# tlepoint/fhe.rs

Hardware: NVIDIA H100
Metric: bfv_ct_mul_relin_per_sec_n32768_14x62bit (higher is better)
Workload: dtype u64

## Files before the change

fhe_rs_b200/_capi.py:

```python
from __future__ import annotations

import ctypes as C
import os

_HERE = os.path.dirname(os.path.abspath(__file__))
LIB_PATH = os.environ.get("FHE_B200_LIB") or os.path.join(_HERE, "libfhe_b200.so")

OK = 0
INVALID_ARGUMENT, INVALID_MODULUS, INVALID_DEGREE, NTT_UNAVAILABLE = -1, -2, -3, -4
CONTEXT_MISMATCH, INVALID_LEVEL, BAD_POLY_COUNT, INVALID_REPRESENTATION = -5, -6, -7, -8
NO_MORE_CONTEXT, INVALID_EXPONENT, UNSUPPORTED = -9, -10, -11
CUDA_ERROR, OUT_OF_MEMORY, NO_DEVICE = -20, -21, -22
POWER_BASIS, NTT = 0, 1
ENCODING_POLY, ENCODING_SIMD = 0, 1

_u32, _u64, _vp, _i = C.c_uint32, C.c_uint64, C.c_void_p, C.c_int
_pu32, _pu64, _pu8 = C.POINTER(C.c_uint32), C.POINTER(C.c_uint64), C.POINTER(C.c_uint8)
_pp = C.POINTER(C.c_void_p)
SYMBOLS = {
    "fhe_b200_version": (C.c_char_p, []),
    "fhe_b200_last_error": (C.c_char_p, []),
    "fhe_b200_params_create": (_i, [_i, _u32, _vp, _u32, _vp, _u32, _vp, _pp]),
    "fhe_b200_params_create_from_sizes": (_i, [_i, _u32, _vp, _u32, _vp, _u32, _pp]),
    "fhe_b200_params_destroy": (_i, [_vp]),
# ... 67 lines not shown
    "fhe_b200_expand": (_i, [_vp, _u32, _pp, _u32, _vp, _vp]),
    "fhe_b200_substitute": (_i, [_vp, _u32, _vp, _vp]),
    "fhe_b200_switch_down": (_i, [_vp, _vp]),
    "fhe_b200_key_switch": (_i, [_vp, _u32, _vp, _vp, _vp]),
    "fhe_b200_key_switch_keyed": (_i, [_vp, _u32, _pp, _u32, _pu32, _vp, _vp]),
    "fhe_b200_relinearize_keyed": (_i, [_vp, _pp, _u32, _pu32, _vp, _vp]),
    "fhe_b200_mul_relin_keyed": (_i, [_vp, _vp, _pp, _u32, _pu32, _i, _vp, _vp]),
    "fhe_b200_galois_keyed": (_i, [_vp, _u32, _pp, _u32, _pu32, _vp, _vp]),
    "fhe_b200_expand_keyed": (_i, [_vp, _u32, _pp, _u32, _u32, _pu32, _vp, _vp]),
    "fhe_b200_galois_many": (_i, [_vp, _pu32, _pp, _pu32, _u32, _pu32, _vp, _vp]),
    "fhe_b200_inner_sum": (_i, [_vp, _pp, _u32, _vp, _vp]),
    "fhe_b200_inner_sum_keyed": (_i, [_vp, _pp, _u32, _u32, _pu32, _vp, _vp]),
    "fhe_b200_scale": (_i, [_vp, _i, _vp, _vp]),
    "fhe_b200_poly_packed_bytes": (_i, [_vp, _u32, C.POINTER(C.c_size_t)]),
    "fhe_b200_batch_packed_bytes": (_i, [_vp, C.POINTER(C.c_size_t)]),
    "fhe_b200_batch_pack": (_i, [_vp, _u32, _u32, _vp, _vp]),
    "fhe_b200_batch_unpack": (_i, [_vp, _u32, _u32, _vp, _vp]),
    "fhe_b200_transcode": (_i, [_vp, _vp, _u32, C.c_size_t, C.c_size_t, _u32, _vp, _u32, C.c_size_t, C.c_size_t,
                                _u32, _u32, _vp]),
    "fhe_b200_fold": (_i, [_vp, _u32, _u32, _vp, _vp]),
    "fhe_b200_sync": (_i, [_vp]),
    "fhe_b200_launch_count": (_u64, []),
    "fhe_b200_debug_scaler_tables": (_i, [_vp, _u32, _i, _pu32, _pu32, _pu32] + [_vp] * 8),
    "fhe_b200_debug_ntt_tables": (_i, [_vp, _u64, _vp, _vp, _vp, _vp, _pu64]),
    "fhe_b200_debug_expansion_monomial": (_i, [_vp, _u32, _u32, _vp]),
    "fhe_b200_debug_encoder_tables": (_i, [_vp, _u32, _vp, _vp, _vp, _pu64, _vp]),
}

_lib = None


def lib() -> C.CDLL:
    global _lib
    if _lib is None:
        if not os.path.exists(LIB_PATH):
            raise ImportError(
                "fhe_rs_b200: %s is missing -- build it with `python -m fhe_rs_b200.build` "
                "(there is no CPU fallback)" % LIB_PATH)
        _lib = C.CDLL(LIB_PATH)
        for name, (res, args) in SYMBOLS.items():
            f = getattr(_lib, name)
            f.restype, f.argtypes = res, args
    return _lib


class FheError(RuntimeError):
# ... 9 lines not shown
```

fhe_rs_b200/csrc/capi.cu:

```cuda
#include <algorithm>
#include <atomic>
#include <cstring>
#include <functional>
#include <map>
#include <memory>
#include <mutex>
#include <string>
#include <vector>

#include "../../include/fhe_b200.h"
#include "engine.hpp"
#include "host/precompute.hpp"

using namespace fhe_b200;

namespace {

thread_local std::string g_last_error;

struct ScalerData {
  ScalerTablesH h;
  ScalerDev dev;
};

// ... 76 lines not shown
  d.tg_lo = s.h.theta_gamma_lo; d.tg_hi = s.h.theta_gamma_hi; d.tg_sign = s.h.theta_gamma_sign;
  for (size_t j = 0; j < to_moduli.size(); j++) d.to_ids[j] = (unsigned short)prime_index(limb_primes, to_moduli[j]);
  d.all_solinas = switches().no_solinas ? 0 : 1;
  for (u64 q : to_moduli)
    if ((q >> 61) != 1 || ((1ull << 62) - q) >= (1ull << 28)) d.all_solinas = 0;
  d.gamma = tables.put(s.h.gamma);
  d.omega = tables.put(s.h.omega);
  d.to_lo = tables.put(s.h.theta_omega_lo);
  d.to_hi = tables.put(s.h.theta_omega_hi);
  d.to_sign = tables.put(s.h.theta_omega_sign);
  std::vector<unsigned char> order;
  d.n_pos = 0;
  for (int sg = 0; sg < 2; sg++)
    for (size_t i = 0; i < s.h.theta_omega_sign.size(); i++)
      if ((int)s.h.theta_omega_sign[i] == sg && (s.h.theta_omega_lo[i] | s.h.theta_omega_hi[i]) != 0) {
        order.push_back((unsigned char)i);
        d.n_pos += sg == 0;
      }
  d.n_terms = (u32)order.size();
  if (order.empty()) order.push_back(0);
  d.to_order = tables.put(order);
  d.tgar_lo = tables.put(s.h.theta_garner_lo);
  d.tgar_hi = tables.put(s.h.theta_garner_hi);
}

LimbDev make_limb_dev(u64 q, const NttTablesH& t, DeviceTables& tables) {
  ModulusH m(q);
  LimbDev d;
  std::memset(&d, 0, sizeof(d));
  d.p = q; d.p2 = 2 * q; d.bhi = m.bhi; d.blo = m.blo; d.c128 = m.c128;
  d.ninv = t.ninv; d.zn = t.zn;
  const u64 cc = (1ull << 62) - q;
  const bool sol = (q >> 61) == 1 && cc < (1ull << 28) && !switches().no_solinas;
  const bool sol_ntt = switches().solinas_ntt;
  auto pairs = [&](const std::vector<u64>& v, const std::vector<u64>& shoup) {
    std::vector<ulonglong2> o(v.size());
    for (size_t k = 0; k < v.size(); k++) {
      o[k].x = v[k];
      o[k].y = (sol && sol_ntt) ? (u64)((((u128)v[k]) << 32) % q) : shoup[k];
    }
    return o;
  };
  d.sol_c = sol ? cc : 0;
  d.sol_ntt = (sol && sol_ntt) ? 1 : 0;
  d.ninv_s = (sol && sol_ntt) ? (u64)((((u128)t.ninv) << 32) % q) : t.ninv_s;
  d.zn_s = (sol && sol_ntt) ? (u64)((((u128)t.zn) << 32) % q) : t.zn_s;
// ... 463 lines not shown
}

void galois_range(const fhe_b200_params* par, const LevelData& lv, const KeySet& gk, const u64* src, u32 src0, u64* dst,
                  u32 n, bool sum, cudaStream_t st) {
  const size_t row = (size_t)1 << par->logn, L = lv.L;
  std::vector<u32> exps(n), source(n);
  for (u32 c = 0; c < n; c++) {
    exps[c] = gk.exps[gk.key_of(c)];
    source[c] = gk.source ? gk.source[c] : src0 + c;
  }
  Workspace ws(par, st);
  u64* s = sum ? nullptr : ws.words((size_t)n * 2 * L * row);
  u64* c2 = ws.words((size_t)n * L * row);
  launch_substitute_ntt(src, 2 * L * row, sum ? dst : s, 2 * L * row, c2, L * row, exps.data(), source.data(), n,
                        (u32)L, sum, lv.ctx_ids, par->d_limbs, par->logn, st);
  launch_ntt(c2, c2, n * (u32)L, lv.ctx_ids, par->d_limbs, par->logn, true, 1, false, st);
  key_switch_apply(par, gk, c2, n, dst, sum ? 1 : 2, s, ws, st);
}

void mul_core(const fhe_b200_params* par, const LevelData& lv, const u64* a, const u64* b, u32 cts, u64* out0,
              u64* out1, int split, Workspace& ws, cudaStream_t st) {
  const u32 L = lv.L, E = lv.E, K = lv.K, logn = par->logn;
  const size_t row = (size_t)1 << logn;
  u64* A_l = ws.words((size_t)cts * 2 * L * row);
  u64* A_r = ws.words((size_t)cts * 2 * L * row);
  u64* X_l = ws.words((size_t)cts * 2 * E * row);
  u64* X_r = ws.words((size_t)cts * 2 * E * row);
  u64* T = ws.words((size_t)cts * 3 * K * row);
  launch_ntt(a, A_l, cts * 2 * L, lv.ctx_ids, par->d_limbs, logn, true, 1, false, st);
  launch_ntt(b, A_r, cts * 2 * L, lv.ctx_ids, par->d_limbs, logn, true, 1, false, st);
  launch_scale(lv.ext.dev, par->d_limbs, A_l, X_l, nullptr, cts * 2, E, L, E, 0, logn, st);
  launch_scale(lv.ext.dev, par->d_limbs, A_r, X_r, nullptr, cts * 2, E, L, E, 0, logn, st);
  launch_ntt(X_l, X_l, cts * 2 * E, lv.ext_ids, par->d_limbs, logn, false, 1, false, st);
  launch_ntt(X_r, X_r, cts * 2 * E, lv.ext_ids, par->d_limbs, logn, false, 1, false, st);
  if (!launch_tensor_inverse_ntt(a, b, X_l, X_r, T, cts, L, K, lv.mul_ids, par->d_limbs, logn, st)) {
    launch_tensor(a, b, X_l, X_r, T, cts, L, L, L, K, lv.mul_ids, par->d_limbs, logn, st);
    launch_ntt(T, T, cts * 3 * K, lv.mul_ids, par->d_limbs, logn, true, 1, false, st);
  }
  launch_scale(lv.down.dev, par->d_limbs, T, out0, out1, cts * 3, L, 0, L, split, logn, st);
}

void mul_core_parts(const fhe_b200_params* par, const LevelData& lv, const u64* a, u32 na, const u64* b, u32 nb, u32 cts,
                    u64* out, Workspace& ws, cudaStream_t st) {
  const u32 L = lv.L, E = lv.E, K = lv.K, logn = par->logn, nc = na + nb - 1;
  const size_t row = (size_t)1 << logn;
  const u64* src[2] = {a, b};
  const u32 np[2] = {na, nb};
  u64* X[2];
  for (int s = 0; s < 2; s++) {
    u64* pb = ws.words((size_t)cts * np[s] * L * row);
    X[s] = ws.words((size_t)cts * np[s] * E * row);
    launch_ntt(src[s], pb, cts * np[s] * L, lv.ctx_ids, par->d_limbs, logn, true, 1, false, st);
    launch_scale(lv.ext.dev, par->d_limbs, pb, X[s], nullptr, cts * np[s], E, L, E, 0, logn, st);
    launch_ntt(X[s], X[s], cts * np[s] * E, lv.ext_ids, par->d_limbs, logn, false, 1, false, st);
  }
  u64* T = ws.words((size_t)cts * nc * K * row);
  launch_tensor_nm(a, b, X[0], X[1], T, cts, L, E, na, nb, lv.mul_ids, par->d_limbs, logn, st);
// ... 2224 lines not shown
  const LevelData& lv = par->level(out->level);
  const u32 L = lv.L, logn = par->logn, count = ct->count;
  ChunkRunner chunks(par, count, (cudaStream_t)stream, std::max<u32>(1, chunk_size() / (u32)P));
  chunks.run([&](u32 c0, u32 n, cudaStream_t st) {
    Workspace ws(par, st);
    u64* coeffs = ws.words((P * n) << logn);
    launch_fold_stage(ct->d + c0 * ct->words_per_ct(), n, ct->parts, row_words, in_bits, out_bits, (u32)P, coeffs, logn,
                      st);
    for (size_t i = 0; i < P; i++)
      launch_ntt(coeffs + ((i * n) << logn), out->d + ((i * count + c0) * L << logn), n * L, lv.ctx_ids, par->d_limbs,
                 logn, false, L, true, st);
  });
  FHE_CUDA(cudaGetLastError());
  out->repr = FHE_B200_NTT;
  API_END
}

int fhe_b200_sync(void* stream) {
  API_BEGIN
  FHE_CUDA(cudaStreamSynchronize((cudaStream_t)stream));
  API_END
}

int fhe_b200_debug_scaler_tables(const fhe_b200_params* p, uint32_t level, int which, uint32_t* n_from, uint32_t* n_to,
                                 uint32_t* shift, uint64_t* gamma, uint64_t* omega, uint64_t* theta_gamma,
                                 uint64_t* theta_omega_lo, uint64_t* theta_omega_hi, uint8_t* theta_omega_sign,
                                 uint64_t* theta_garner_lo, uint64_t* theta_garner_hi) {
  API_BEGIN
  REQUIRE(p, FHE_B200_INVALID_ARGUMENT, "null argument");
  const LevelData& lv = p->level(level);
  REQUIRE(which >= 0 && which <= 2, FHE_B200_INVALID_ARGUMENT, "which must be 0, 1 or 2");
  const ScalerTablesH& h = which == 0 ? lv.ext.h : which == 1 ? lv.down.h : lv.plain.h;
  if (n_from) *n_from = h.n_from;
  if (n_to) *n_to = h.n_to;
  if (shift) *shift = h.shift;
  auto cp = [](uint64_t* dst, const std::vector<u64>& v) {
    if (dst) for (size_t i = 0; i < v.size(); i++) dst[i] = v[i];
  };
  cp(gamma, h.gamma);
  cp(omega, h.omega);
  if (theta_gamma) { theta_gamma[0] = h.theta_gamma_lo; theta_gamma[1] = h.theta_gamma_hi; theta_gamma[2] = h.theta_gamma_sign; }
  cp(theta_omega_lo, h.theta_omega_lo);
  cp(theta_omega_hi, h.theta_omega_hi);
  if (theta_omega_sign) for (size_t i = 0; i < h.theta_omega_sign.size(); i++) theta_omega_sign[i] = h.theta_omega_sign[i];
  cp(theta_garner_lo, h.theta_garner_lo);
  cp(theta_garner_hi, h.theta_garner_hi);
// ... 52 lines not shown
```

fhe_rs_b200/csrc/engine.hpp:

```cpp
#pragma once
#include <atomic>
#include <cuda.h>
#include <cuda_runtime.h>
#include <vector>

#include "ntt.cuh"

namespace fhe_b200 {

extern std::atomic<unsigned long long> g_launches;

struct Switches {
  enum Ntt { NTT_FAST, NTT_AUTO, NTT_TMA };
  enum Ksmac { KSMAC_FUSED, KSMAC_TMA, KSMAC_CLASSIC };
  u32 chunk;
  u32 streams;
  Ntt ntt;
  bool generic_ntt;
  bool solinas_ntt;
  bool no_solinas;
  bool no_tensor_fusion;
  bool classic_scaler;
  Ksmac ksmac;
  int tma_cols;
// ... 48 lines not shown
void launch_dot(const u64* ct, const u64* pt, u64* out, u32 groups, u32 n_terms, u32 parts, u32 ct_count,
                u32 pt_count, const RowIds& ids, const LimbDev* limbs, u32 logn, cudaStream_t st);

void launch_tensor(const u64* a, const u64* b, const u64* xa, const u64* xb, u64* out, u32 cts, u32 L, u32 nca,
                   u32 ncb, u32 K, const RowIds& mul_ids, const LimbDev* limbs, u32 logn, cudaStream_t st);

void launch_tensor_nm(const u64* a, const u64* b, const u64* xa, const u64* xb, u64* out, u32 cts, u32 L, u32 E, u32 na,
                      u32 nb, const RowIds& mul_ids, const LimbDev* limbs, u32 logn, cudaStream_t st);

struct ScalerDev {
  u32 n_from, n_to, is_one, shift;
  u64 tg_lo, tg_hi;
  u32 tg_sign;
  u32 all_solinas;
  const u64* gamma;
  const u64* omega;
  const u64* to_lo;
  const u64* to_hi;
  const unsigned char* to_sign;
  const unsigned char* to_order;
  u32 n_pos, n_terms;
  const u64* tgar_lo;
  const u64* tgar_hi;
  unsigned short to_ids[kMaxPos];
};
void launch_scale(const ScalerDev& S, const LimbDev* limbs, const u64* in, u64* out0, u64* out1, u32 polys,
                  u32 out_rows_per_poly, u32 start, u32 n_out, int split3, u32 logn, cudaStream_t st);

constexpr u32 kKeyPairs = 64;
constexpr u32 kKeySlots = 512;
struct KeyTable {
  const u64* k0[kKeyPairs];
  const u64* k1[kKeyPairs];
  u32 n;
  unsigned char slot[kKeySlots];
};
struct KeyRange {
  u32 ct0, cts;
  KeyTable keys;
};
#ifdef __CUDACC__
__device__ __forceinline__ u32 key_slot(const KeyTable& K, u32 ct) { return K.n > 1 ? K.slot[ct] : 0; }
#endif

void launch_ksmac(const u64* inter, const std::vector<KeyRange>& ranges, const u64* base0, const u64* base1, u64* out0,
                  u64* out1, u32 n_dig, u32 Lk, u32 out_ct_rows, const RowIds& ids, const LimbDev* limbs, u32 logn,
                  cudaStream_t st, bool adjacent = false);

// ... 96 lines not shown
```

fhe_rs_b200/csrc/host/precompute.hpp:

```cpp
#pragma once
#include <cstdint>
#include <stdexcept>
#include <string>
#include <vector>

#include "bigint.hpp"

namespace fhe_b200 {

typedef unsigned long long u64;
typedef unsigned __int128 u128;

struct FheError : std::runtime_error {
  int code;
  FheError(int c, const std::string& m) : std::runtime_error(m), code(c) {}
};

inline u64 mulmod_h(u64 a, u64 b, u64 p) { return (u64)((u128)a * b % p); }
inline u64 powmod_h(u64 a, u64 e, u64 p) {
  u64 r = 1 % p;
  a %= p;
  while (e) {
    if (e & 1) r = mulmod_h(r, a, p);
    a = mulmod_h(a, a, p);
// ... 107 lines not shown
  BigUint product;
  std::vector<BigUint> garner;
  explicit RnsContextH(const std::vector<u64>& q) : moduli(q), product(1) {
    if (q.empty()) throw FheError(-2, "EmptyModuli");
    for (u64 m : q) product = product * BigUint(m);
    for (u64 m : q) {
      BigUint q_star = product / BigUint(m);
      u64 q_tilde;
      if (!invmod_h(q_star.mod_u64(m), m, &q_tilde)) throw FheError(-2, "NonCoprimeModuli");
      garner.push_back(q_star * BigUint(q_tilde));
    }
  }
};

struct ScalerTablesH {
  uint32_t n_from = 0, n_to = 0, is_one = 0, shift = 0;
  std::vector<u64> gamma;
  u64 theta_gamma_lo = 0, theta_gamma_hi = 0;
  uint32_t theta_gamma_sign = 0;
  std::vector<u64> omega;
  std::vector<u64> theta_omega_lo, theta_omega_hi;
  std::vector<uint8_t> theta_omega_sign;
  std::vector<u64> theta_garner_lo, theta_garner_hi;
};

inline void extract_projection_and_theta(const std::vector<u64>& to, const BigUint& input, const BigUint& num,
                                         const BigUint& den, bool round_up, std::vector<u64>* projected,
                                         u64* lo, u64* hi, bool* sign) {
  BigUint ni = num * input;
  BigUint gamma = (ni + (den >> 1)) / den;
  projected->clear();
  for (u64 m : to) projected->push_back(gamma.mod_u64(m));
  BigUint theta = ni % den;
  bool s = false;
  if (den > BigUint(1)) {
    if (den.is_odd()) {
      if (theta > (den >> 1)) { s = true; theta = den - theta; }
    } else if (theta >= (den >> 1)) { s = true; theta = den - theta; }
  }
  if (round_up) {
    theta = s ? (theta << 127) / den : ((theta << 127) + den - BigUint(1)) / den;
  } else {
    theta = s ? ((theta << 127) + den - BigUint(1)) / den : (theta << 127) / den;
  }
  u128 v = theta.low_u128();
  *lo = (u64)v;
// ... 1 lines not shown
  *sign = s;
}

inline ScalerTablesH make_scaler_tables(const RnsContextH& from, const RnsContextH& to, const BigUint& num,
                                        const BigUint& den) {
  if (den.is_zero()) throw FheError(-1, "scaling factor denominator is zero");
  ScalerTablesH t;
  t.n_from = (uint32_t)from.moduli.size();
  t.n_to = (uint32_t)to.moduli.size();
  t.is_one = num == den;
  bool sg;
  extract_projection_and_theta(to.moduli, from.product, num, den, false, &t.gamma, &t.theta_gamma_lo,
                               &t.theta_gamma_hi, &sg);
  t.theta_gamma_sign = sg;
  t.omega.assign((size_t)t.n_to * t.n_from, 0);
  t.theta_omega_lo.resize(t.n_from);
  t.theta_omega_hi.resize(t.n_from);
  t.theta_omega_sign.resize(t.n_from);
  for (uint32_t i = 0; i < t.n_from; i++) {
    std::vector<u64> proj;
    extract_projection_and_theta(to.moduli, from.garner[i], num, den, true, &proj, &t.theta_omega_lo[i],
                                 &t.theta_omega_hi[i], &sg);
    t.theta_omega_sign[i] = sg;
    for (uint32_t j = 0; j < t.n_to; j++) t.omega[(size_t)j * t.n_from + i] = proj[j] % to.moduli[j];
  }
  uint32_t shift = 127;
  for (u64 qi : from.moduli) {
    u128 v = (u128)qi * t.n_from;
    uint32_t lg = 0;
    while (((u128)1 << lg) < v) lg++;
    uint32_t s = 192 - 1 - lg;
    if (s < shift) shift = s;
  }
  t.shift = shift;
  t.theta_garner_lo.resize(t.n_from);
  t.theta_garner_hi.resize(t.n_from);
  for (uint32_t i = 0; i < t.n_from; i++) {
    BigUint theta = ((from.garner[i] << shift) + (from.product >> 1)) / from.product;
    u128 v = theta.low_u128();
    t.theta_garner_lo[i] = (u64)v;
    t.theta_garner_hi[i] = (u64)(v >> 64);
  }
  return t;
}

}
```

fhe_rs_b200/csrc/kernels.cu:

```cuda
#include <algorithm>
#include <cstdint>
#include <cstdlib>
#include <cstring>
#include <vector>

#include "engine.hpp"
#include "ntt_tma.cuh"

namespace fhe_b200 {

typedef unsigned __int128 u128;

namespace {

struct EwArgs {
  u64* a;
  const u64* b;
  size_t n_words;
  u32 logn, limbs_per_poly;
  const LimbDev* limbs;
  unsigned short ids[kMaxPos];
};

template <int OP>
// ... 387 lines not shown
      u64 y = acc[k].reduce(M);
      u64* dst;
      if (A.split3) {
        u32 ct = poly / 3, part = poly % 3;
        dst = part < 2 ? A.out0 + ((((size_t)ct * 2 + part) * n_out + jj) << A.logn)
                       : A.out1 + (((size_t)ct * n_out + jj) << A.logn);
      } else {
        dst = A.out0 + (((size_t)poly * A.out_rows_per_poly + jj) << A.logn);
      }
      dst[c0 + cc] = y;
    }
  }
}


struct ScaleTmaArgs {
  ScalerDev S;
  const LimbDev* limbs;
  u64 *out0, *out1;
  u32 polys, out_rows_per_poly, start, n_out, split3, logn;
  u32 tiles_total;
};

template <bool IS_ONE, int UNR>
__global__ void __launch_bounds__(kScaleTC) scale_tma_kernel(const __grid_constant__ CUtensorMap tm_in, const ScaleTmaArgs A) {
  using namespace tma;
  extern __shared__ __align__(128) u64 smem[];
  const ScalerDev& S = A.S;
  const u32 nf = S.n_from, n_out = A.n_out;
  const u32 n_out4 = (n_out + 3) & ~3u;
  constexpr u32 TC = kScaleTC;
  u64* s_r = smem;
  u32* s_omega = reinterpret_cast<u32*>(s_r + (size_t)nf * TC);
  u64* s_gamma = reinterpret_cast<u64*>(s_omega + (size_t)nf * 3 * n_out4);
  u64* s_p2 = s_gamma + n_out4;
  u64* s_c = s_p2 + n_out4;
  u64* s_tgl = s_c + n_out4;
  u64* s_tgh = s_tgl + nf;
  u64* s_tol = s_tgh + nf;
  u64* s_toh = s_tol + nf;
  u32* s_ord = reinterpret_cast<u32*>(s_toh + nf);
  u64* s_bar = reinterpret_cast<u64*>(s_ord + ((nf + 1) & ~1u));
  const u32 bar = smem_u32(s_bar);
  const u32 cc = threadIdx.x;

  stage_omega_split(s_omega, S, A.start, n_out, n_out4);
  for (u32 i = cc; i < n_out4; i += TC) {
    const bool live = i < n_out;
    const LimbDev& M = A.limbs[S.to_ids[A.start + (live ? i : 0)]];
    s_gamma[i] = live ? S.gamma[A.start + i] : 0;
    s_p2[i] = M.p2;
    s_c[i] = M.sol_c;
  }
  for (u32 i = cc; i < nf; i += TC) {
    s_tgl[i] = S.tgar_lo[i];
    s_tgh[i] = S.tgar_hi[i];
    const u32 src = (!IS_ONE && i < S.n_terms) ? S.to_order[i] : 0;
    s_tol[i] = IS_ONE ? 0 : S.to_lo[src];
    s_toh[i] = IS_ONE ? 0 : S.to_hi[src];
    s_ord[i] = src * TC * 8;
  }
  if (cc == 0) {
    mbar_init(bar, 1);
    asm volatile("fence.mbarrier_init.release.cluster;" ::: "memory");
  }
  __syncthreads();

  const u32 N = 1u << A.logn;
  const u32 per_poly = N / TC;
  const u32 dst_r = smem_u32(s_r);
  const u32 tile_bytes = nf * TC * 8;
  u32 tile = blockIdx.x;
  if (cc == 0 && tile < A.tiles_total) {
    mbar_expect_tx(bar, tile_bytes);
    load_2d(dst_r, &tm_in, (tile % per_poly) * TC, (tile / per_poly) * nf, bar);
  }
  const u32 my_r = dst_r + cc * 8;
  for (u32 it = 0; tile < A.tiles_total; tile += gridDim.x, it++) {
    const u32 poly = tile / per_poly;
    const u32 c0 = (tile - poly * per_poly) * TC;
    mbar_wait(bar, it & 1);

    u128 v;
    {
      AccTheta at;
      at.clear();
#pragma unroll 2
      for (u32 i = 0; i < nf; i++) at.mac(lds64(my_r + i * TC * 8), s_tgl[i], s_tgh[i]);
      u32 acc[7];
      at.words(acc);
      U256 sg = u256_from_acc(acc);
      const u32 bs = S.shift - 1 - 64;
      u64 lo = (sg.w1 >> bs) | (sg.w2 << (64 - bs));
      u64 hi = (sg.w2 >> bs) | (sg.w3 << (64 - bs));
      u128 x = ((u128)hi << 64) | lo;
      v = (x >> 1) + (x & 1);
    }
    bool w_sign = false;
    u128 w = 0;
    if (!IS_ONE) {
      U256 s_pos = {0, 0, 0, 0}, s_neg = {0, 0, 0, 0};
#pragma unroll 1
      for (u32 sg = 0; sg < 2; sg++) {
        AccTheta at;
        at.clear();
        const u32 k0 = sg ? S.n_pos : 0, k1 = sg ? S.n_terms : S.n_pos;
#pragma unroll 2
        for (u32 k = k0; k < k1; k++) at.mac(lds64(my_r + s_ord[k]), s_tol[k], s_toh[k]);
        u32 wds[7];
        at.words(wds);
        if (sg == 0) s_pos = u256_from_acc(wds);
        else s_neg = u256_from_acc(wds);
      }
      U256 so = u256_sub(s_pos, s_neg);
      U256 vt = u256_mul_128(v, S.tg_lo, S.tg_hi);
      so = S.tg_sign ? u256_add(so, vt) : u256_sub(so, vt);
      w_sign = (so.w3 != 0) || (so.w2 >> 63);
      if (w_sign) {
        u64 n1 = ~so.w1, n2 = ~so.w2, n3 = ~so.w3;
        u128 y = ((u128)((n2 >> 62) | (n3 << 2)) << 64) | ((n1 >> 62) | (n2 << 2));
        w = (y + 1) >> 1;
      } else {
        u128 y = ((u128)((so.w2 >> 62) | (so.w3 << 2)) << 64) | ((so.w1 >> 62) | (so.w2 << 2));
        w = (y >> 1) + (y & 1);
      }
    }
    const u64 mask62 = (1ull << 62) - 1;
    const u64 vl = (u64)v & mask62, wl = (u64)w & mask62;
    const u32 vh = (u32)(v >> 62), wh = (u32)(w >> 62);

    u64* dst;
    size_t dstride = (size_t)1 << A.logn;
    if (A.split3) {
      const u32 ct = poly / 3, part = poly - ct * 3;
      dst = part < 2 ? A.out0 + ((((size_t)ct * 2 + part) * n_out) << A.logn) : A.out1 + (((size_t)ct * n_out) << A.logn);
    } else {
      dst = A.out0 + (((size_t)poly * A.out_rows_per_poly) << A.logn);
    }
    dst += c0 + cc;

    for (u32 j0 = 0; j0 < n_out; j0 += 4) {
      AccKara acc[4];
#pragma unroll
      for (int k = 0; k < 4; k++) acc[k].clear();
      const u32* om = s_omega + j0;
      const u32 g = min(4u, n_out - j0);
      switch (g) {
        case 4: scale_mac_group<4, UNR>(acc, s_r + cc, om, nf, n_out4); break;
        case 3: scale_mac_group<3, UNR>(acc, s_r + cc, om, nf, n_out4); break;
        case 2: scale_mac_group<2, UNR>(acc, s_r + cc, om, nf, n_out4); break;
// ... 7 lines not shown
          load_2d(dst_r, &tm_in, (nxt % per_poly) * TC, (nxt / per_poly) * nf, bar);
        }
      }
#pragma unroll
      for (int k = 0; k < 4; k++) {
        const u32 jj = j0 + k;
        if (jj >= n_out) break;
        const u64 p2 = s_p2[jj];
        const u32 c = (u32)s_c[jj];
        acc[k].mac(split31(csub(p2 - ((u64)vh * c + vl), p2 >> 1)), split31(s_gamma[jj]));
        if (!IS_ONE) {
          const u64 wr = (u64)wh * c + wl;
          acc[k].add64(w_sign ? p2 - wr : wr);
        }
        u64 lo, mid;
        u32 hi32;
        acc[k].merged(lo, mid, hi32);
        dst[(size_t)jj * dstride] = csub(fold192_solinas(lo, mid, hi32, c), p2 >> 1);
      }
    }
  }
}

__global__ void scale_small_kernel(ScaleArgs A) {
  const ScalerDev& S = A.S;
  const u32 nf = S.n_from, n_out = A.n_out;
  const u32 N = 1u << A.logn;
  const u32 idx = blockIdx.x * blockDim.x + threadIdx.x;
  if (idx >= A.polys * N) return;
  const u32 poly = idx >> A.logn, c = idx & (N - 1);
  const u64* src = A.in + (((size_t)poly * nf) << A.logn) + c;
  u32 av[7] = {0, 0, 0, 0, 0, 0, 0}, ap[7] = {0, 0, 0, 0, 0, 0, 0}, an[7] = {0, 0, 0, 0, 0, 0, 0};
  for (u32 i = 0; i < nf; i++) {
    const u64 r = src[(size_t)i << A.logn];
    mac_theta(av, r, S.tgar_lo[i], S.tgar_hi[i]);
    if (!S.is_one) {
      if (S.to_sign[i]) mac_theta(an, r, S.to_lo[i], S.to_hi[i]);
      else mac_theta(ap, r, S.to_lo[i], S.to_hi[i]);
    }
  }
  U256 sg = u256_from_acc(av);
  const u32 bs = S.shift - 1 - 64;
  u64 lo = (sg.w1 >> bs) | (sg.w2 << (64 - bs));
  u64 hi = (sg.w2 >> bs) | (sg.w3 << (64 - bs));
  u128 x = ((u128)hi << 64) | lo;
  u128 v = (x >> 1) + (x & 1);
// ... 1080 lines not shown
  A.cts = cts; A.L = L; A.E = E; A.na = na; A.nb = nb; A.logn = logn;
  A.limbs = limbs;
  copy_ids(A.ids, mul_ids);
  size_t total = ((size_t)cts * (na + nb - 1) * (L + E)) << logn;
  if (!total) return;
  tensor_nm_kernel<<<(unsigned)((total + 255) / 256), 256, 0, st>>>(A);
  g_launches++;
}

static bool launch_scale_tma(const ScalerDev& S, const LimbDev* limbs, const u64* in, u64* out0, u64* out1, u32 polys,
                             u32 out_rows_per_poly, u32 start, u32 n_out, int split3, u32 logn, cudaStream_t st) {
  if (switches().classic_scaler || !tensor_map_encoder() || logn < 7 || (reinterpret_cast<uintptr_t>(in) & 127))
    return false;
  const u32 N = 1u << logn, nf = S.n_from;
  if (nf > 64 || (u64)polys * nf >= (1ull << 31)) return false;
  CUtensorMap tm;
  if (!box_map(&tm, in, (u64)polys * nf, logn, kScaleTC, nf)) return false;
  ScaleTmaArgs A;
  A.S = S; A.limbs = limbs; A.out0 = out0; A.out1 = out1;
  A.polys = polys; A.out_rows_per_poly = out_rows_per_poly; A.start = start; A.n_out = n_out;
  A.split3 = split3; A.logn = logn;
  A.tiles_total = polys * (N / kScaleTC);
  const size_t n_out4 = (n_out + 3) & ~(size_t)3;
  const size_t smem = (nf * kScaleTC + 3 * n_out4 + 4 * nf) * sizeof(u64) + nf * 3 * n_out4 * sizeof(u32) +
                      ((nf + 1) & ~(size_t)1) * 4 + 16;
  auto resident = [&](const void* k) {
    ensure_dynamic_smem(k, smem);
    int per_sm = 0;
    FHE_CUDA(cudaOccupancyMaxActiveBlocksPerMultiprocessor(&per_sm, k, kScaleTC, smem));
    return (u32)std::min<u64>(A.tiles_total, (u64)sm_count() * std::max(per_sm, 1));
  };
  if (switches().scale_unroll == 4) {
    if (S.is_one) scale_tma_kernel<true, 4><<<resident((const void*)scale_tma_kernel<true, 4>), kScaleTC, smem, st>>>(tm, A);
    else scale_tma_kernel<false, 4><<<resident((const void*)scale_tma_kernel<false, 4>), kScaleTC, smem, st>>>(tm, A);
  } else {
    if (S.is_one) scale_tma_kernel<true, 2><<<resident((const void*)scale_tma_kernel<true, 2>), kScaleTC, smem, st>>>(tm, A);
    else scale_tma_kernel<false, 2><<<resident((const void*)scale_tma_kernel<false, 2>), kScaleTC, smem, st>>>(tm, A);
  }
  g_launches++;
  return true;
}

void launch_scale(const ScalerDev& S, const LimbDev* limbs, const u64* in, u64* out0, u64* out1, u32 polys,
                  u32 out_rows_per_poly, u32 start, u32 n_out, int split3, u32 logn, cudaStream_t st) {
  if (!polys || !n_out) return;
  if (S.all_solinas &&
      launch_scale_tma(S, limbs, in, out0, out1, polys, out_rows_per_poly, start, n_out, split3, logn, st))
    return;
  ScaleArgs A;
  A.S = S; A.limbs = limbs; A.in = in; A.out0 = out0; A.out1 = out1;
  A.polys = polys; A.out_rows_per_poly = out_rows_per_poly; A.start = start; A.n_out = n_out;
  A.split3 = split3; A.logn = logn;
  const u32 N = 1u << logn;
  if (N < (u32)kScaleTC) {
    const u32 total = polys * N;
    scale_small_kernel<<<(total + 63) / 64, 64, 0, st>>>(A);
    g_launches++;
    return;
  }
  const size_t n_out4 = (n_out + 3) & ~(size_t)3, nf = S.n_from;
  const size_t smem = (nf * kScaleTC + n_out4 + 5 * nf) * sizeof(u64) + nf * 3 * n_out4 * sizeof(u32);
  ensure_dynamic_smem((const void*)scale_kernel, smem);
  scale_kernel<<<polys * (N / kScaleTC), kScaleTC, smem, st>>>(A);
// ... 168 lines not shown
```

include/fhe_b200.h:

```cpp
#ifndef FHE_B200_H
#define FHE_B200_H

#include <stddef.h>
#include <stdint.h>

#ifdef __cplusplus
extern "C" {
#endif

typedef enum {
  FHE_B200_OK = 0,
  FHE_B200_INVALID_ARGUMENT = -1,
  FHE_B200_INVALID_MODULUS = -2,
  FHE_B200_INVALID_DEGREE = -3,
  FHE_B200_NTT_UNAVAILABLE = -4,
  FHE_B200_CONTEXT_MISMATCH = -5,
  FHE_B200_INVALID_LEVEL = -6,
  FHE_B200_BAD_POLY_COUNT = -7,
  FHE_B200_INVALID_REPRESENTATION = -8,
  FHE_B200_NO_MORE_CONTEXT = -9,
  FHE_B200_INVALID_EXPONENT = -10,
  FHE_B200_UNSUPPORTED = -11,
  FHE_B200_CUDA_ERROR = -20,
  FHE_B200_OUT_OF_MEMORY = -21,
// ... 156 lines not shown
                             const uint32_t* set_index, fhe_b200_batch* out, void* stream);
int fhe_b200_scale(const fhe_b200_batch* in, int which, fhe_b200_batch* out, void* stream);
int fhe_b200_batch_alloc_mul_basis(const fhe_b200_params* p, uint32_t count, uint32_t parts, uint32_t level,
                                   int repr, fhe_b200_batch** out);

int fhe_b200_poly_packed_bytes(const fhe_b200_params* p, uint32_t level, size_t* nbytes);
int fhe_b200_batch_packed_bytes(const fhe_b200_batch* b, size_t* nbytes);
int fhe_b200_batch_pack(const fhe_b200_batch* b, uint32_t first, uint32_t n, uint8_t* host_out, void* stream);
int fhe_b200_batch_unpack(fhe_b200_batch* b, uint32_t first, uint32_t n, const uint8_t* host_in, void* stream);

int fhe_b200_transcode(const fhe_b200_params* p, const void* in, uint32_t in_elem, size_t in_len, size_t in_stride,
                       uint32_t in_bits, void* out, uint32_t out_elem, size_t out_len, size_t out_stride,
                       uint32_t out_bits, uint32_t n_rows, void* stream);
int fhe_b200_fold(const fhe_b200_batch* ct, uint32_t in_bits, uint32_t out_bits, fhe_b200_batch* out, void* stream);

int fhe_b200_sync(void* stream);
uint64_t fhe_b200_launch_count(void);

int fhe_b200_debug_scaler_tables(const fhe_b200_params* p, uint32_t level, int which, uint32_t* n_from,
                                 uint32_t* n_to, uint32_t* shift, uint64_t* gamma, uint64_t* omega,
                                 uint64_t* theta_gamma , uint64_t* theta_omega_lo,
                                 uint64_t* theta_omega_hi, uint8_t* theta_omega_sign,
                                 uint64_t* theta_garner_lo, uint64_t* theta_garner_hi);
int fhe_b200_debug_ntt_tables(const fhe_b200_params* p, uint64_t q, uint64_t* omegas, uint64_t* omegas_shoup,
                              uint64_t* zetas_inv, uint64_t* zetas_inv_shoup, uint64_t* size_inv);
int fhe_b200_debug_expansion_monomial(const fhe_b200_params* p, uint32_t level, uint32_t l, uint64_t* out);
int fhe_b200_debug_encoder_tables(const fhe_b200_encoder* e, uint32_t level, uint32_t* index_map, uint64_t* omegas,
                                  uint64_t* zetas_inv, uint64_t* q_mod_t, uint64_t* delta);

#ifdef __cplusplus
}
#endif
#endif
```

Baseline: 3831.

## Use Karatsuba-split accumulation with float fractional estimate in TMA scaler, exact fallback

The TMA scaler kernels now accumulate the truncated top part of the Garner and omega theta constants with a 31-bit split Karatsuba accumulator. The low bits are estimated with a double-precision FMA, and the full 128-bit AccTheta path runs only when the fractional part falls within a precomputed error bound of the rounding boundary. Fallbacks are counted in a device atomic, and the down-scaling kernel gets its own instantiation with different launch bounds. Separately, the left and right extension scale and NTT launches are merged into single launches over contiguous buffers. This trades wide multiplies for cheaper arithmetic, at the cost of more shared memory and a rare divergent exact path.

```diff
diff --git a/fhe_rs_b200/_capi.py b/fhe_rs_b200/_capi.py
--- a/fhe_rs_b200/_capi.py
+++ b/fhe_rs_b200/_capi.py
@@ -113,6 +113,7 @@
     "fhe_b200_sync": (_i, [_vp]),
     "fhe_b200_launch_count": (_u64, []),
     "fhe_b200_debug_scaler_tables": (_i, [_vp, _u32, _i, _pu32, _pu32, _pu32] + [_vp] * 8),
+    "fhe_b200_debug_scaler_fallbacks": (_i, [_pu64]),
     "fhe_b200_debug_ntt_tables": (_i, [_vp, _u64, _vp, _vp, _vp, _vp, _pu64]),
     "fhe_b200_debug_expansion_monomial": (_i, [_vp, _u32, _u32, _vp]),
     "fhe_b200_debug_encoder_tables": (_i, [_vp, _u32, _vp, _vp, _vp, _pu64, _vp]),
diff --git a/fhe_rs_b200/csrc/capi.cu b/fhe_rs_b200/csrc/capi.cu
--- a/fhe_rs_b200/csrc/capi.cu
+++ b/fhe_rs_b200/csrc/capi.cu
@@ -122,6 +122,12 @@
   d.to_order = tables.put(order);
   d.tgar_lo = tables.put(s.h.theta_garner_lo);
   d.tgar_hi = tables.put(s.h.theta_garner_hi);
+  d.tgar_top = tables.put(s.h.theta_garner_top);
+  d.tgar_bot = tables.put(s.h.theta_garner_bot);
+  d.v_eps = s.h.v_eps;
+  d.to_top = tables.put(s.h.theta_omega_top);
+  d.to_bot = tables.put(s.h.theta_omega_bot);
+  d.w_eps = s.h.w_eps;
 }
 
 LimbDev make_limb_dev(u64 q, const NttTablesH& t, DeviceTables& tables) {
@@ -631,17 +637,15 @@
               u64* out1, int split, Workspace& ws, cudaStream_t st) {
   const u32 L = lv.L, E = lv.E, K = lv.K, logn = par->logn;
   const size_t row = (size_t)1 << logn;
-  u64* A_l = ws.words((size_t)cts * 2 * L * row);
-  u64* A_r = ws.words((size_t)cts * 2 * L * row);
-  u64* X_l = ws.words((size_t)cts * 2 * E * row);
-  u64* X_r = ws.words((size_t)cts * 2 * E * row);
+  u64* A_l = ws.words((size_t)cts * 4 * L * row);
+  u64* A_r = A_l + (size_t)cts * 2 * L * row;
+  u64* X_l = ws.words((size_t)cts * 4 * E * row);
+  u64* X_r = X_l + (size_t)cts * 2 * E * row;
   u64* T = ws.words((size_t)cts * 3 * K * row);
   launch_ntt(a, A_l, cts * 2 * L, lv.ctx_ids, par->d_limbs, logn, true, 1, false, st);
   launch_ntt(b, A_r, cts * 2 * L, lv.ctx_ids, par->d_limbs, logn, true, 1, false, st);
-  launch_scale(lv.ext.dev, par->d_limbs, A_l, X_l, nullptr, cts * 2, E, L, E, 0, logn, st);
-  launch_scale(lv.ext.dev, par->d_limbs, A_r, X_r, nullptr, cts * 2, E, L, E, 0, logn, st);
-  launch_ntt(X_l, X_l, cts * 2 * E, lv.ext_ids, par->d_limbs, logn, false, 1, false, st);
-  launch_ntt(X_r, X_r, cts * 2 * E, lv.ext_ids, par->d_limbs, logn, false, 1, false, st);
+  launch_scale(lv.ext.dev, par->d_limbs, A_l, X_l, nullptr, cts * 4, E, L, E, 0, logn, st);
+  launch_ntt(X_l, X_l, cts * 4 * E, lv.ext_ids, par->d_limbs, logn, false, 1, false, st);
   if (!launch_tensor_inverse_ntt(a, b, X_l, X_r, T, cts, L, K, lv.mul_ids, par->d_limbs, logn, st)) {
     launch_tensor(a, b, X_l, X_r, T, cts, L, L, L, K, lv.mul_ids, par->d_limbs, logn, st);
     launch_ntt(T, T, cts * 3 * K, lv.mul_ids, par->d_limbs, logn, true, 1, false, st);
@@ -2912,6 +2916,13 @@
   API_END
 }
 
+int fhe_b200_debug_scaler_fallbacks(uint64_t* count) {
+  API_BEGIN
+  REQUIRE(count, FHE_B200_INVALID_ARGUMENT, "null argument");
+  *count = scale_fallbacks();
+  API_END
+}
+
 int fhe_b200_debug_scaler_tables(const fhe_b200_params* p, uint32_t level, int which, uint32_t* n_from, uint32_t* n_to,
                                  uint32_t* shift, uint64_t* gamma, uint64_t* omega, uint64_t* theta_gamma,
                                  uint64_t* theta_omega_lo, uint64_t* theta_omega_hi, uint8_t* theta_omega_sign,
diff --git a/fhe_rs_b200/csrc/engine.hpp b/fhe_rs_b200/csrc/engine.hpp
--- a/fhe_rs_b200/csrc/engine.hpp
+++ b/fhe_rs_b200/csrc/engine.hpp
@@ -94,8 +94,15 @@
   u32 n_pos, n_terms;
   const u64* tgar_lo;
   const u64* tgar_hi;
+  const u64* tgar_top;
+  const double* tgar_bot;
+  double v_eps;
+  const u64* to_top;
+  const double* to_bot;
+  double w_eps;
   unsigned short to_ids[kMaxPos];
 };
+unsigned long long scale_fallbacks();
 void launch_scale(const ScalerDev& S, const LimbDev* limbs, const u64* in, u64* out0, u64* out1, u32 polys,
                   u32 out_rows_per_poly, u32 start, u32 n_out, int split3, u32 logn, cudaStream_t st);
 
diff --git a/fhe_rs_b200/csrc/host/precompute.hpp b/fhe_rs_b200/csrc/host/precompute.hpp
--- a/fhe_rs_b200/csrc/host/precompute.hpp
+++ b/fhe_rs_b200/csrc/host/precompute.hpp
@@ -1,4 +1,5 @@
 #pragma once
+#include <cmath>
 #include <cstdint>
 #include <stdexcept>
 #include <string>
@@ -153,6 +154,12 @@
   std::vector<u64> theta_omega_lo, theta_omega_hi;
   std::vector<uint8_t> theta_omega_sign;
   std::vector<u64> theta_garner_lo, theta_garner_hi;
+  std::vector<u64> theta_garner_top;
+  std::vector<double> theta_garner_bot;
+  double v_eps = 0;
+  std::vector<u64> theta_omega_top;
+  std::vector<double> theta_omega_bot;
+  double w_eps = 0;
 };
 
 inline void extract_projection_and_theta(const std::vector<u64>& to, const BigUint& input, const BigUint& num,
@@ -200,6 +207,10 @@
     extract_projection_and_theta(to.moduli, from.garner[i], num, den, true, &proj, &t.theta_omega_lo[i],
                                  &t.theta_omega_hi[i], &sg);
     t.theta_omega_sign[i] = sg;
+    const u128 th = ((u128)t.theta_omega_hi[i] << 64) | t.theta_omega_lo[i];
+    t.theta_omega_top.push_back((u64)(th >> 66));
+    const double bot = std::ldexp((double)(th & (((u128)1 << 66) - 1)), 31 - 126);
+    t.theta_omega_bot.push_back(sg ? -bot : bot);
     for (uint32_t j = 0; j < t.n_to; j++) t.omega[(size_t)j * t.n_from + i] = proj[j] % to.moduli[j];
   }
   uint32_t shift = 127;
@@ -218,6 +229,22 @@
     u128 v = theta.low_u128();
     t.theta_garner_lo[i] = (u64)v;
     t.theta_garner_hi[i] = (u64)(v >> 64);
+    t.theta_garner_top.push_back((u64)(v >> 66));
+    t.theta_garner_bot.push_back(std::ldexp((double)(v & (((u128)1 << 66) - 1)), 31 - (int)shift));
+  }
+  {
+    const double n = t.n_from, lmax = std::ldexp(n, 128 - (int)shift);
+    int e = 0;
+    while (std::ldexp(1.0, e) < lmax + 2) e++;
+    t.v_eps = 2 * (std::ldexp(n, 97 - (int)shift) + std::ldexp(lmax, -53) + std::ldexp(n + 1, e - 54) +
+                   std::ldexp(1.0, -54));
+  }
+  {
+    const double n = t.n_from, lmax = 4 * n;
+    int e = 0;
+    while (std::ldexp(1.0, e) < lmax + 2) e++;
+    t.w_eps = 2 * (std::ldexp(n, -29) + std::ldexp(lmax, -53) + std::ldexp(n + 1, e - 54) + std::ldexp(1.0, -62) +
+                   std::ldexp(1.0, -54) + std::ldexp(1.0, -53));
   }
   return t;
 }
diff --git a/fhe_rs_b200/csrc/kernels.cu b/fhe_rs_b200/csrc/kernels.cu
--- a/fhe_rs_b200/csrc/kernels.cu
+++ b/fhe_rs_b200/csrc/kernels.cu
@@ -433,8 +433,10 @@
   u32 tiles_total;
 };
 
+__device__ unsigned long long g_scale_fallbacks = 0;
+
 template <bool IS_ONE, int UNR>
-__global__ void __launch_bounds__(kScaleTC) scale_tma_kernel(const __grid_constant__ CUtensorMap tm_in, const ScaleTmaArgs A) {
+__device__ __forceinline__ void scale_tma_body(const CUtensorMap& tm_in, const ScaleTmaArgs& A) {
   using namespace tma;
   extern __shared__ __align__(128) u64 smem[];
   const ScalerDev& S = A.S;
@@ -448,9 +450,11 @@
   u64* s_c = s_p2 + n_out4;
   u64* s_tgl = s_c + n_out4;
   u64* s_tgh = s_tgl + nf;
-  u64* s_tol = s_tgh + nf;
-  u64* s_toh = s_tol + nf;
-  u32* s_ord = reinterpret_cast<u32*>(s_toh + nf);
+  uint4* s_gk = reinterpret_cast<uint4*>(s_tgh + nf);
+  uint4* s_wk = s_gk + nf;
+  double* s_gb = reinterpret_cast<double*>(s_wk + nf);
+  double* s_wb = s_gb + nf;
+  u32* s_ord = reinterpret_cast<u32*>(s_wb + nf);
   u64* s_bar = reinterpret_cast<u64*>(s_ord + ((nf + 1) & ~1u));
   const u32 bar = smem_u32(s_bar);
   const u32 cc = threadIdx.x;
@@ -467,9 +471,13 @@
     s_tgl[i] = S.tgar_lo[i];
     s_tgh[i] = S.tgar_hi[i];
     const u32 src = (!IS_ONE && i < S.n_terms) ? S.to_order[i] : 0;
-    s_tol[i] = IS_ONE ? 0 : S.to_lo[src];
-    s_toh[i] = IS_ONE ? 0 : S.to_hi[src];
     s_ord[i] = src * TC * 8;
+    const Split31 g = split31(S.tgar_top[i]);
+    s_gk[i] = make_uint4(g.lo, g.hi, g.sum, 0);
+    s_gb[i] = S.tgar_bot[i];
+    const Split31 o = split31(IS_ONE ? 0 : S.to_top[src]);
+    s_wk[i] = make_uint4(o.lo, o.hi, o.sum, 0);
+    s_wb[i] = IS_ONE ? 0.0 : S.to_bot[src];
   }
   if (cc == 0) {
     mbar_init(bar, 1);
@@ -491,41 +499,97 @@
     const u32 poly = tile / per_poly;
     const u32 c0 = (tile - poly * per_poly) * TC;
     mbar_wait(bar, it & 1);
+    const u64 mask62 = (1ull << 62) - 1;
 
     u128 v;
     {
-      AccTheta at;
-      at.clear();
+      AccKara ak;
+      ak.clear();
+      double lf = 0.0;
 #pragma unroll 2
-      for (u32 i = 0; i < nf; i++) at.mac(lds64(my_r + i * TC * 8), s_tgl[i], s_tgh[i]);
-      u32 acc[7];
-      at.words(acc);
-      U256 sg = u256_from_acc(acc);
-      const u32 bs = S.shift - 1 - 64;
-      u64 lo = (sg.w1 >> bs) | (sg.w2 << (64 - bs));
-      u64 hi = (sg.w2 >> bs) | (sg.w3 << (64 - bs));
-      u128 x = ((u128)hi << 64) | lo;
-      v = (x >> 1) + (x & 1);
+      for (u32 i = 0; i < nf; i++) {
+        const Split31 r = split31(lds64(my_r + i * TC * 8));
+        const uint4 g = s_gk[i];
+        ak.mac(r.lo, r.hi, r.sum, g.x, g.y, g.z);
+        lf = fma(__hiloint2double(0x43300000, (int)r.hi) - 0x1p52, s_gb[i], lf);
+      }
+      u64 lo, mid;
+      u32 hi;
+      ak.merged(lo, mid, hi);
+      const u32 d = S.shift - 66;
+      const u128 h_int = ((u128)((mid >> d) | ((u64)hi << (64 - d))) << 64) | ((lo >> d) | (mid << (64 - d)));
+      const double z = __ull2double_rn(lo & ((1ull << d) - 1)) * __longlong_as_double((long long)(1023 - d) << 52) + lf;
+      const double k = floor(z), fr = z - k;
+      if (fabs(fr - 0.5) > S.v_eps) {
+        v = h_int + (u64)k + (fr > 0.5);
+      } else {
+        atomicAdd(&g_scale_fallbacks, 1ull);
+        AccTheta at;
+        at.clear();
+        for (u32 i = 0; i < nf; i++) at.mac(lds64(my_r + i * TC * 8), s_tgl[i], s_tgh[i]);
+        u32 acc[7];
+        at.words(acc);
+        U256 sg = u256_from_acc(acc);
+        const u32 bs = S.shift - 1 - 64;
+        u64 xl = (sg.w1 >> bs) | (sg.w2 << (64 - bs));
+        u64 xh = (sg.w2 >> bs) | (sg.w3 << (64 - bs));
+        u128 x = ((u128)xh << 64) | xl;
+        v = (x >> 1) + (x & 1);
+      }
     }
     bool w_sign = false;
     u128 w = 0;
     if (!IS_ONE) {
-      U256 s_pos = {0, 0, 0, 0}, s_neg = {0, 0, 0, 0};
+      U256 so, s_pos = {0, 0, 0, 0}, s_neg = {0, 0, 0, 0};
+      double wf = 0.0;
 #pragma unroll 1
       for (u32 sg = 0; sg < 2; sg++) {
-        AccTheta at;
-        at.clear();
+        AccKara ak;
+        ak.clear();
         const u32 k0 = sg ? S.n_pos : 0, k1 = sg ? S.n_terms : S.n_pos;
 #pragma unroll 2
-        for (u32 k = k0; k < k1; k++) at.mac(lds64(my_r + s_ord[k]), s_tol[k], s_toh[k]);
-        u32 wds[7];
-        at.words(wds);
-        if (sg == 0) s_pos = u256_from_acc(wds);
-        else s_neg = u256_from_acc(wds);
+        for (u32 k = k0; k < k1; k++) {
+          const Split31 r = split31(lds64(my_r + s_ord[k]));
+          const uint4 g = s_wk[k];
+          ak.mac(r.lo, r.hi, r.sum, g.x, g.y, g.z);
+          wf = fma(__hiloint2double(0x43300000, (int)r.hi) - 0x1p52, s_wb[k], wf);
+        }
+        u64 lo, mid;
+        u32 hi;
+        ak.merged(lo, mid, hi);
+        const U256 t = {lo, mid, hi, 0};
+        if (sg == 0) s_pos = t;
+        else s_neg = t;
       }
-      U256 so = u256_sub(s_pos, s_neg);
-      U256 vt = u256_mul_128(v, S.tg_lo, S.tg_hi);
-      so = S.tg_sign ? u256_add(so, vt) : u256_sub(so, vt);
+      const U256 d = u256_sub(s_pos, s_neg);
+      U256 x = {0, d.w0 << 2, (d.w1 << 2) | (d.w0 >> 62), (d.w2 << 2) | (d.w1 >> 62)};
+      const U256 vt = u256_mul_128(v, S.tg_lo, S.tg_hi);
+      x = S.tg_sign ? u256_add(x, vt) : u256_sub(x, vt);
+      const double z = __ull2double_rn(x.w1 & mask62) * 0x1p-62 + wf;
+      const double k = floor(z), fr = z - k;
+      if (fr > S.w_eps && fr < 1.0 - S.w_eps) {
+        const long long kk = (long long)k;
+        const U256 kx = {0, (u64)kk << 62, (u64)(kk >> 2), (u64)(kk >> 63)};
+        so = u256_add({0, x.w1 & ~mask62, x.w2, x.w3}, kx);
+      } else {
+        atomicAdd(&g_scale_fallbacks, 1ull);
+#pragma unroll 1
+        for (u32 sg = 0; sg < 2; sg++) {
+          AccTheta at;
+          at.clear();
+          const u32 k0 = sg ? S.n_pos : 0, k1 = sg ? S.n_terms : S.n_pos;
+          for (u32 k = k0; k < k1; k++) {
+            const u32 src = S.to_order[k];
+            at.mac(lds64(my_r + s_ord[k]), S.to_lo[src], S.to_hi[src]);
+          }
+          u32 wds[7];
+          at.words(wds);
+          if (sg == 0) s_pos = u256_from_acc(wds);
+          else s_neg = u256_from_acc(wds);
+        }
+        so = u256_sub(s_pos, s_neg);
+        so = S.tg_sign ? u256_add(so, vt) : u256_sub(so, vt);
+      }
       w_sign = (so.w3 != 0) || (so.w2 >> 63);
       if (w_sign) {
         u64 n1 = ~so.w1, n2 = ~so.w2, n3 = ~so.w3;
@@ -536,7 +600,6 @@
         w = (y >> 1) + (y & 1);
       }
     }
-    const u64 mask62 = (1ull << 62) - 1;
     const u64 vl = (u64)v & mask62, wl = (u64)w & mask62;
     const u32 vh = (u32)(v >> 62), wh = (u32)(w >> 62);
 
@@ -590,6 +653,16 @@
   }
 }
 
+template <bool IS_ONE, int UNR>
+__global__ void __launch_bounds__(kScaleTC) scale_tma_kernel(const __grid_constant__ CUtensorMap tm_in, const ScaleTmaArgs A) {
+  static_assert(IS_ONE, "");
+  scale_tma_body<true, UNR>(tm_in, A);
+}
+template <int UNR>
+__global__ void __launch_bounds__(kScaleTC, UNR == 2 ? 6 : 1) scale_tma_down_kernel(const __grid_constant__ CUtensorMap tm_in, const ScaleTmaArgs A) {
+  scale_tma_body<false, UNR>(tm_in, A);
+}
+
 __global__ void scale_small_kernel(ScaleArgs A) {
   const ScalerDev& S = A.S;
   const u32 nf = S.n_from, n_out = A.n_out;
@@ -1716,7 +1789,7 @@
   A.split3 = split3; A.logn = logn;
   A.tiles_total = polys * (N / kScaleTC);
   const size_t n_out4 = (n_out + 3) & ~(size_t)3;
-  const size_t smem = (nf * kScaleTC + 3 * n_out4 + 4 * nf) * sizeof(u64) + nf * 3 * n_out4 * sizeof(u32) +
+  const size_t smem = (nf * kScaleTC + 3 * n_out4 + 8 * nf) * sizeof(u64) + nf * 3 * n_out4 * sizeof(u32) +
                       ((nf + 1) & ~(size_t)1) * 4 + 16;
   auto resident = [&](const void* k) {
     ensure_dynamic_smem(k, smem);
@@ -1726,13 +1799,19 @@
   };
   if (switches().scale_unroll == 4) {
     if (S.is_one) scale_tma_kernel<true, 4><<<resident((const void*)scale_tma_kernel<true, 4>), kScaleTC, smem, st>>>(tm, A);
-    else scale_tma_kernel<false, 4><<<resident((const void*)scale_tma_kernel<false, 4>), kScaleTC, smem, st>>>(tm, A);
+    else scale_tma_down_kernel<4><<<resident((const void*)scale_tma_down_kernel<4>), kScaleTC, smem, st>>>(tm, A);
   } else {
     if (S.is_one) scale_tma_kernel<true, 2><<<resident((const void*)scale_tma_kernel<true, 2>), kScaleTC, smem, st>>>(tm, A);
-    else scale_tma_kernel<false, 2><<<resident((const void*)scale_tma_kernel<false, 2>), kScaleTC, smem, st>>>(tm, A);
+    else scale_tma_down_kernel<2><<<resident((const void*)scale_tma_down_kernel<2>), kScaleTC, smem, st>>>(tm, A);
   }
   g_launches++;
   return true;
+}
+
+unsigned long long scale_fallbacks() {
+  unsigned long long n = 0;
+  FHE_CUDA(cudaMemcpyFromSymbol(&n, g_scale_fallbacks, sizeof(n)));
+  return n;
 }
 
 void launch_scale(const ScalerDev& S, const LimbDev* limbs, const u64* in, u64* out0, u64* out1, u32 polys,
diff --git a/include/fhe_b200.h b/include/fhe_b200.h
--- a/include/fhe_b200.h
+++ b/include/fhe_b200.h
@@ -202,6 +202,7 @@
                                  uint64_t* theta_gamma , uint64_t* theta_omega_lo,
                                  uint64_t* theta_omega_hi, uint8_t* theta_omega_sign,
                                  uint64_t* theta_garner_lo, uint64_t* theta_garner_hi);
+int fhe_b200_debug_scaler_fallbacks(uint64_t* count);
 int fhe_b200_debug_ntt_tables(const fhe_b200_params* p, uint64_t q, uint64_t* omegas, uint64_t* omegas_shoup,
                               uint64_t* zetas_inv, uint64_t* zetas_inv_shoup, uint64_t* size_inv);
 int fhe_b200_debug_expansion_monomial(const fhe_b200_params* p, uint32_t level, uint32_t l, uint64_t* out);
diff --git a/profiles/scaler_bench.py b/profiles/scaler_bench.py
--- /dev/null
+++ b/profiles/scaler_bench.py
@@ -0,0 +1,110 @@
+import argparse
+import json
+import os
+import subprocess
+import sys
+
+DEGREE, PLAINTEXT, N_MODULI = 1 << 15, 786433, 14
+
+
+def worker(args):
+    sys.path.insert(0, args.tree)
+    import numpy as np
+    import torch
+    from torch.profiler import ProfilerActivity, profile
+    import bench
+    import fhe_rs_b200 as F
+    from fhe_rs_b200._capi import check
+    L = F._capi.lib()
+    par = F.BfvParameters(DEGREE, PLAINTEXT, moduli_sizes=[62] * N_MODULI, device=0)
+    moduli = par.moduli()
+    B = args.batch
+    A, Bt, out = F.Ciphertext(par, B, 2), F.Ciphertext(par, B, 2), F.Ciphertext(par, B, 2)
+    bench.fill_uniform(torch, A, moduli, 1)
+    bench.fill_uniform(torch, Bt, moduli, 2)
+    rng = np.random.default_rng(7)
+    kc = np.zeros((2, N_MODULI, N_MODULI, DEGREE), np.uint64)
+    for i, q in enumerate(moduli):
+        kc[:, :, i, :] = rng.integers(0, q, size=(2, N_MODULI, DEGREE), dtype=np.uint64)
+    rk = F.RelinearizationKey.from_arrays(par, kc[0], kc[1])
+
+    def step():
+        check(L.fhe_b200_mul_relin(A._h, Bt._h, rk.ksk._h, 0, out._h, None))
+
+    for _ in range(3):
+        step()
+    torch.cuda.synchronize()
+    e0, e1 = torch.cuda.Event(enable_timing=True), torch.cuda.Event(enable_timing=True)
+    e0.record()
+    for _ in range(args.steps):
+        step()
+    e1.record()
+    torch.cuda.synchronize()
+    mul_us = e0.elapsed_time(e1) * 1e3 / (args.steps * B)
+
+    with profile(activities=[ProfilerActivity.CUDA]) as prof:
+        for _ in range(args.steps):
+            step()
+        torch.cuda.synchronize()
+    sums = {"ext": [0.0, 0], "down": [0.0, 0]}
+    for ka in prof.key_averages():
+        if "scale_tma_kernel" not in ka.key and "scale_tma_down_kernel" not in ka.key:
+            continue
+        kind = "ext" if "scale_tma_kernel<true" in ka.key else "down"
+        sums[kind][0] += getattr(ka, "device_time_total", None) or getattr(ka, "cuda_time_total", 0.0)
+        sums[kind][1] += ka.count
+    n = args.steps * B
+    print(json.dumps({
+        "batch": B, "steps": args.steps,
+        "ext_us_per_product": sums["ext"][0] / n, "ext_launches_per_step": sums["ext"][1] / args.steps,
+        "down_us_per_product": sums["down"][0] / n, "down_launches_per_step": sums["down"][1] / args.steps,
+        "multiply_us_per_product": mul_us,
+    }))
+
+
+def card():
+    try:
+        r = subprocess.run(["nvidia-smi", "--query-gpu=name,power.limit,clocks.sm,clocks.max.sm",
+                            "--format=csv,noheader"], capture_output=True, text=True, timeout=30)
+        return r.stdout.strip().splitlines()[0]
+    except Exception as e:
+        return "unread (%s)" % e
+
+
+def main():
+    ap = argparse.ArgumentParser()
+    ap.add_argument("--trees", nargs="+", default=["this=."], help="label=path, one per build to compare")
+    ap.add_argument("--rounds", type=int, default=3)
+    ap.add_argument("--batch", type=int, default=256)
+    ap.add_argument("--steps", type=int, default=10)
+    ap.add_argument("--out")
+    ap.add_argument("--worker", action="store_true")
+    ap.add_argument("--tree", default=".")
+    args = ap.parse_args()
+    if args.worker:
+        return worker(args)
+    trees = [t.split("=", 1) for t in args.trees]
+    rows = []
+    for rnd in range(args.rounds):
+        for label, path in trees:
+            r = subprocess.run([sys.executable, os.path.abspath(__file__), "--worker", "--tree", os.path.abspath(path),
+                                "--batch", str(args.batch), "--steps", str(args.steps)],
+                               capture_output=True, text=True, check=True)
+            row = json.loads(r.stdout.strip().splitlines()[-1])
+            row.update(label=label, round=rnd, card=card())
+            rows.append(row)
+            print(json.dumps(row), flush=True)
+    summary = {}
+    for label, _ in trees:
+        mine = [r for r in rows if r["label"] == label]
+        summary[label] = {k: [round(r[k], 3) for r in mine]
+                          for k in ("ext_us_per_product", "down_us_per_product", "multiply_us_per_product",
+                                    "ext_launches_per_step", "down_launches_per_step")}
+    print(json.dumps({"summary": summary, "card": card()}, indent=1))
+    if args.out:
+        with open(args.out, "w") as f:
+            json.dump({"rows": rows, "summary": summary}, f, indent=1)
+
+
+if __name__ == "__main__":
+    main()
```

After: 3871, median of 6. 1.01x the previous value.
